# Da1yuqin/TCDiff

Hardware: AMD Instinct MI355X
Metric: sampled clips/sec (3 dancers x 150 frames, 1000 DDPM steps) (higher is better)
Workload: dtype bf16; 1 GPU; batch=16 clips/GPU, 3 dancers x 150 frames, 1000 DDPM steps (p_sample_loop, CFG w=2, cosine schedule), bf16, 1xMI355X; clips_per_gpu=16, ddpm_steps=1000

## Files before the change

include/tcdiff_hip.h:

```cpp
#ifndef TCDIFF_HIP_H
#define TCDIFF_HIP_H

#include <stdint.h>

#ifdef __cplusplus
extern "C" {
#endif

#ifndef __HIP__
typedef struct ihipStream_t* hipStream_t;
#endif

#define TCDIFF_OK 0
#define TCDIFF_ERR_ARG (-1)
#define TCDIFF_ERR_ALIGN (-2)
#define TCDIFF_ERR_LAUNCH (-3)
#define TCDIFF_ERR_UNSUPPORTED (-4)

#define TC_DTYPE_F32 0
#define TC_DTYPE_BF16 1
#define TC_DTYPE_BF16X3 2

#define TC_ACT_NONE 0
#define TC_ACT_RELU 1
// ... 6 lines not shown
#define TC_EPI_QKV_HEADS 2
#define TC_EPI_ATOMIC_F32 3

typedef struct {
    int mode;
    int act;
    float scale_q;
    const float* bias;
    void* out;
    void* out_k;
    void* out_v;
    int ldc;
    int L, Lp, H;
    int n_q, n_k;
    int tok_off;
    int seq_off;
    int k_splits;
    void* out2; int ldc2;
    const void* act_src; int ld_src;
    int act2;
    const int* drop_seed; int drop_site; uint32_t drop_thr; float drop_scale;
    int hgroup; long hgroup_stride;
    int small_m;
} tcdiff_tile_epi;

int tcdiff_gemm_tile(int dtype, const void* A, const void* A2, int split_n, const void* W, int M, int N, int K,
                     int lda, int ldw, int a_mod, const tcdiff_tile_epi* epi, hipStream_t stream);

#define TC_ROW_BIAS 1
#define TC_ROW_LN_POST 2
#define TC_ROW_FILM 4
#define TC_ROW_RES 8
#define TC_ROW_STORE_X 16
#define TC_ROW_NEXT_LN 32
#define TC_ROW_STORE_H 64
#define TC_ROW_STORE_ROT 128

typedef struct {
    int flags;
    const float* bias;
    const float* ln_g;
    const float* ln_b;
    float ln_eps;
    const float* film;
    int film_ld;
    const float* xres;
    int xres_mod;
// ... 433 lines not shown
```

tcdiff_amd/_lib.py:

```python
import ctypes as C
import os

HERE = os.path.dirname(os.path.abspath(__file__))
LIB_PATH = os.environ.get("TCDIFF_LIB_PATH") or os.path.join(HERE, "libtcdiff_gfx950.so")

DT_F32, DT_BF16, DT_BF16X3 = 0, 1, 2
ACT_NONE, ACT_RELU, ACT_GELU, ACT_MISH, ACT_SILU = 0, 1, 2, 3, 4
EPI_STORE_T, EPI_STORE_F32, EPI_QKV_HEADS = 0, 1, 2
ROW_BIAS, ROW_LN_POST, ROW_FILM, ROW_RES, ROW_STORE_X, ROW_NEXT_LN, ROW_STORE_H, ROW_STORE_ROT = \
    1, 2, 4, 8, 16, 32, 64, 128
SAMPLER_DDPM, SAMPLER_DDIM = 0, 1
EXPORT_NORMAL, EXPORT_LONG = 0, 1
SAMPLER_ADVANCE = 0x100
CHAIN_A, CHAIN_B, CHAIN_B_LAST, CHAIN_FULL, CHAIN_FULL_LAST, CHAIN_FRONT = 0, 1, 2, 3, 4, 5

_vp, _i, _f, _l = C.c_void_p, C.c_int, C.c_float, C.c_long


class TileEpi(C.Structure):
    _fields_ = [("mode", _i), ("act", _i), ("scale_q", _f), ("bias", _vp), ("out", _vp), ("out_k", _vp),
                ("out_v", _vp), ("ldc", _i), ("L", _i), ("Lp", _i), ("H", _i), ("n_q", _i), ("n_k", _i),
                ("tok_off", _i), ("seq_off", _i), ("k_splits", _i), ("out2", _vp), ("ldc2", _i), ("act_src", _vp),
                ("ld_src", _i), ("act2", _i), ("drop_seed", _vp), ("drop_site", _i), ("drop_thr", C.c_uint32),
                ("drop_scale", _f), ("hgroup", _i), ("hgroup_stride", _l), ("small_m", _i)]


class RowEpi(C.Structure):
    _fields_ = [("flags", _i), ("bias", _vp), ("ln_g", _vp), ("ln_b", _vp), ("ln_eps", _f), ("film", _vp),
                ("film_ld", _i), ("xres", _vp), ("xres_mod", _i), ("xout", _vp), ("L", _i), ("nln_g", _vp),
                ("nln_b", _vp), ("nln_eps", _f), ("hout", _vp), ("rout", _vp), ("rope", _vp), ("out_mul", _i),
                ("out_add", _i), ("groups", _i)]


class ChainArgs(C.Structure):
    _fields_ = [("mode", _i), ("n_stages", _i), ("M", _i), ("L", _i), ("a_mod", _i), ("xres_mod", _i), ("H", _i),
                ("Lp", _i), ("A", _vp), ("wstream", _vp), ("film", _vp), ("xres", _vp),
                ("xout", _vp), ("n2_g", _vp), ("n2_b", _vp), ("rope", _vp), ("q_out", _vp), ("b1", _vp),
                ("film3", _vp), ("n4_g", _vp), ("n4_b", _vp), ("b3", _vp), ("nn_g", _vp), ("nn_b", _vp),
                ("k_out", _vp), ("v_out", _vp), ("h_out", _vp), ("film_ld", _i), ("ln_eps", _f), ("n2_eps", _f),
                ("n4_eps", _f), ("nn_eps", _f), ("scale_q", _f), ("filmb", _vp),
                ("n3_g", _vp), ("n3_b", _vp), ("kf", _vp), ("vf", _vp), ("n_shared", _i), ("nkt", _i), ("Lk", _i),
                ("xres_rowmajor", _i), ("rope_rows", _i), ("dn", _i), ("mt", _i), ("out_ld", _i), ("nw", _i), ("seq_blocks", _i), ("sa_q", _vp), ("sa_kf", _vp), ("sa_vf", _vp),
                ("sa_nkt", _i), ("qf_out", _vp), ("kf_out", _vp), ("vf_out", _vp), ("out_nkt", _i)]


PROLOGUE_X, PROLOGUE_COND = 1, 2

# ... 45 lines not shown
                ("tap_blocks", _vp)]


class NavTrainArgs(C.Structure):
    _fields_ = [("seed0", C.c_uint32), ("seed1", C.c_uint32), ("drop_thr", C.c_uint32), ("drop_scale", _f), ("cond", _vp), ("x_in", _vp)] + \
        [(n, _vp) for n in ("lstm_gates", "lstm_c", "lstm_h", "xs", "xmid", "att_o", "lse", "hid", "dec_z", "mus_z", "d_out", "gx",
                            "g_dec", "g_mpb", "g_m", "g_hid", "g_a", "g_o", "delta", "g_qkv", "n1", "n2", "ln_part", "g_me", "g_mp",
                            "g_mz", "g_gates", "partial", "grads")]


class AdanScalars(C.Structure):
    _fields_ = [(n, _f) for n in ("b1", "omb1", "b2", "omb2", "b3", "omb3", "cm", "cv", "cn", "eps", "lr", "denom")] + \
        [("first", _i)]


class NavAdamWScalars(C.Structure):
    _fields_ = [(n, _f) for n in ("decay", "wd", "omb1", "beta2", "omb2", "neg_step", "bc2_sqrt", "eps")] + [("decoupled", _i)]


NAV_LOSS_BLOCK = 2048

_SIGS = {
    "tcdiff_gemm_tile": [_i, _vp, _vp, _i, _vp, _i, _i, _i, _i, _i, _i, C.POINTER(TileEpi), _vp],
    "tcdiff_gemm_rowln": [_i, _vp, _vp, _i, _i, _i, _i, _i, C.POINTER(RowEpi), _vp],
    "tcdiff_attention": [_i, _vp, _vp, _vp, _vp, _i, _i, _i, _i, _i, _i, _i, _i, _i, _vp],
    "tcdiff_q_sample_traj": [_vp, _vp, _vp, _vp, _vp, _vp, _i, _i, _i, _i, _vp],
    "tcdiff_ax_from_6v": [_vp, _l, _i, _l, _vp, _vp],
    "tcdiff_smpl_fk": [_vp, _vp, _l, C.POINTER(_i), C.POINTER(_f), _vp, _vp],
    "tcdiff_loss_terms": [_vp, _vp, _vp, _vp, _vp, _vp, _vp, _i, _i, _i, _i, _i, _vp],
    "tcdiff_adan_step": [_vp, _i, C.POINTER(AdanScalars), _vp],
    "tcdiff_pack_kv_frags": [_vp, _vp, _vp, _vp, _i, _i, _i, _i, _i, _i, _vp],
    "tcdiff_chain": [C.POINTER(ChainArgs), _vp],
    "tcdiff_chain_split": [C.POINTER(ChainArgs), _i, _vp, _vp, _vp],
    "tcdiff_ln_rot": [_i, _vp, _i, _vp, _vp, _f, _vp, _vp, _vp, _vp, _i, _i, _vp],
    "tcdiff_rope_table": [_vp, _vp, _i, _vp],
    "tcdiff_convert_pad": [_i, _vp, _vp, _i, _i, _i, _i, _l, _l, _vp],
    "tcdiff_sinusoidal": [_i, _vp, _i, _vp, _vp, _vp],
    "tcdiff_mean_pool": [_vp, _vp, _i, _i, _i, _vp],
    "tcdiff_add_act": [_i, _vp, _vp, _vp, _i, _i, _vp, _vp, _vp],
    "tcdiff_scatter_time_kv": [_i, _vp, _i, _vp, _vp, _vp, _i, _i, _i, _i, _i, _vp],
    "tcdiff_step_begin": [_vp, _vp, _vp, _i, _vp],
    "tcdiff_step_end": [_vp, _vp],
    "tcdiff_step_prologue": [_i, _vp, _vp],
    "tcdiff_sampler_update": [_i, _vp, _vp, _i, _vp, _vp, _vp, _vp, _i, _i, _i, _vp, _vp, _vp, C.c_uint64, _i, _vp],
    "tcdiff_window_couple": [_vp, _i, _i, _i, _vp],
    "tcdiff_window_couple_step": [_vp, _i, _i, _i, _vp, _vp, _vp],
# ... 97 lines not shown
```

tcdiff_amd/csrc/gemm.hip:

```cpp
#include "attn_common.h"
#include "train_common.h"
#include "tcdiff_hip.h"

#ifdef TC_STAMP
__device__ unsigned long long* g_tc_stamp = nullptr;
extern "C" int tcdiff_debug_stamp_buffer(void* p) {
    return hipMemcpyToSymbol(HIP_SYMBOL(g_tc_stamp), &p, sizeof(p)) == hipSuccess ? 0 : -1;
}
#define TC_STAMP_AT(i) do { if (tid == 0 && g_tc_stamp) g_tc_stamp[blockIdx.x * 8 + (i)] = __builtin_amdgcn_s_memrealtime(); } while (0)
#define TC_STAMP_W(i) do { if (lane == 0 && g_tc_stamp && (i) < 32) g_tc_stamp[blockIdx.x * 32 + (i)] = __builtin_amdgcn_s_memrealtime(); } while (0)
#else
#define TC_STAMP_AT(i) do { } while (0)
#define TC_STAMP_W(i) do { } while (0)
#endif

template <class P>
DEVINL void unpack_chunk(const u32x4& c, float (&v)[16 / sizeof(typename P::elem_t)]) {
    if (P::IS_BF16) {
#pragma unroll
        for (int j = 0; j < 4; ++j) {
            v[2 * j] = bf2f((uint16_t)(c[j] & 0xffffu));
            v[2 * j + 1] = bf2f((uint16_t)(c[j] >> 16));
        }
    } else {
// ... 692 lines not shown
        const f32x4_t b = *reinterpret_cast<const f32x4_t*>(e.bias + n);
#pragma unroll
        for (int t = 0; t < 4; ++t) v[t] += b[t];
    }
#pragma unroll
    for (int t = 0; t < 4; ++t) v[t] = apply_act(v[t], e.act);
    if (F32OUT) {
        *reinterpret_cast<f32x4_t*>(reinterpret_cast<float*>(e.out) + (long)m * e.ldc + n) = f32x4_t{v[0], v[1], v[2], v[3]};
    } else {
        uint2 pk = {pack_bf2(v[0], v[1]), pack_bf2(v[2], v[3])};
        *reinterpret_cast<uint2*>(reinterpret_cast<uint16_t*>(e.out) + (long)m * e.ldc + n) = pk;
    }
}

static bool small_product(int dtype, const void* A2, int M, int N, int K, const tcdiff_tile_epi& e, int n_cu) {
    static const bool off = [] { const char* v = getenv("TCDIFF_GEMM_SMALL"); return v && v[0] == '0'; }();
    if (off || !e.small_m || dtype != TC_DTYPE_BF16 || A2 || (e.mode != TC_EPI_STORE_T && e.mode != TC_EPI_STORE_F32) || e.out2 || e.act_src)
        return false;
    if (N % 32 || K % 32 || K > 2048 || e.ldc % 4 || (e.bias && !aligned16(e.bias))) return false;
    const long big = (long)((N + 127) / 128) * ((M + 127) / 128), small = (long)(N / 32) * ((M + 31) / 32);
    return big * 4 <= n_cu && small <= 2L * n_cu;
}

static int launch_tile(int dtype, const void* A, const void* A2, int split_n, const void* W, int M, int N, int K,
                       int lda, int ldw, int a_mod, const tcdiff_tile_epi* epi, hipStream_t stream) {
    if (!A || !W || !epi || M <= 0 || N <= 0 || K <= 0) return TC_ERR_ARG;
    if (dtype != TC_DTYPE_BF16 && dtype != TC_DTYPE_F32 && dtype != TC_DTYPE_BF16X3) return TC_ERR_ARG;
    if (dtype == TC_DTYPE_BF16X3 && (epi->mode == TC_EPI_ATOMIC_F32 || epi->out2 || epi->act_src)) return TC_ERR_UNSUPPORTED;
    if (dtype == TC_DTYPE_BF16X3 && epi->mode == TC_EPI_STORE_T && epi->ldc % 4) return TC_ERR_ARG;
    const int es = dtype == TC_DTYPE_BF16 ? 2 : 4;
    const int kt = dtype == TC_DTYPE_BF16 ? 64 : 32;
    if (K % kt != 0) return TC_ERR_ARG;
    if (!aligned16(A) || !aligned16(W) || (A2 && !aligned16(A2)) || ((long)lda * es) % 16 || ((long)ldw * es) % 16)
        return TC_ERR_ALIGN;
    if (A2 && (split_n % 128 != 0)) return TC_ERR_ARG;
    if ((long)(a_mod > 0 ? a_mod : M) * lda * es >= (1L << 32) || (long)N * ldw * es >= (1L << 32)) return TC_ERR_ARG;
    if (epi->bias && !aligned16(epi->bias)) return TC_ERR_ALIGN;
    if (epi->act < TC_ACT_NONE || epi->act > TC_ACT_SILU) return TC_ERR_ARG;
    if (epi->mode == TC_EPI_QKV_HEADS) {
        if (epi->L <= 0 || epi->Lp <= 0 || epi->H <= 0 || epi->n_q % 128 || epi->n_k % 128 || N % 64) return TC_ERR_ARG;
        if ((epi->n_q > 0 && (!epi->out || !aligned16(epi->out))) ||
            (epi->n_k > 0 && (!epi->out_k || !aligned16(epi->out_k))) ||
            (N > epi->n_q + epi->n_k && (!epi->out_v || !aligned16(epi->out_v))))
            return TC_ERR_ALIGN;
    } else {
        if (!epi->out) return TC_ERR_ARG;
// ... 21 lines not shown
        hipError_t err = hipSuccess;
#define TC_TILE_ATTR(POL, ACTK)                                                                                    \
        if (err == hipSuccess)                                                                                     \
            err = hipFuncSetAttribute(reinterpret_cast<const void*>(gemm_tile_kernel<POL, ACTK, 4>),              \
                                      hipFuncAttributeMaxDynamicSharedMemorySize, 4 * 2 * 128 * TC_ROWB);
        TC_TILE_ATTR(MmaBF16, 0) TC_TILE_ATTR(MmaBF16, 1) TC_TILE_ATTR(MmaBF16, 2) TC_TILE_ATTR(MmaBF16, 3)
        TC_TILE_ATTR(MmaF32, 0) TC_TILE_ATTR(MmaF32, 1) TC_TILE_ATTR(MmaF32, 2) TC_TILE_ATTR(MmaF32, 3)
        TC_TILE_ATTR(MmaBF16x3, 0) TC_TILE_ATTR(MmaBF16x3, 1) TC_TILE_ATTR(MmaBF16x3, 2) TC_TILE_ATTR(MmaBF16x3, 3)
#undef TC_TILE_ATTR
        return err;
    });
    if (n_cu < 0) return n_cu;
    if (small_product(dtype, A2, M, N, K, e, n_cu)) {
        const dim3 sgrid((unsigned)((N / 32) * ((M + 31) / 32)));
        if (e.mode == TC_EPI_STORE_F32)
            hipLaunchKernelGGL(gemm_small_kernel<true>, sgrid, dim3(512), 0, stream, (const char*)A, (const char*)W, M, N, K,
                               (long)lda * es, (long)ldw * es, a_mod, e);
        else
            hipLaunchKernelGGL(gemm_small_kernel<false>, sgrid, dim3(512), 0, stream, (const char*)A, (const char*)W, M, N, K,
                               (long)lda * es, (long)ldw * es, a_mod, e);
        TC_CHECK_LAUNCH();
        return TC_OK;
    }
    const bool deep = (long)grid.x * 4 <= (long)n_cu * 5 && K / kt / e.k_splits >= 3;
#define TC_LAUNCH_TILE(POL, ACTK)                                                                                       \
    if (deep)                                                                                                           \
        hipLaunchKernelGGL((gemm_tile_kernel<POL, ACTK, 4>), grid, dim3(256), 4 * 2 * 128 * TC_ROWB, stream,            \
                           (const char*)A, (const char*)A2, split_n, (const char*)W, M, N, K, (long)lda * es,           \
                           (long)ldw * es, a_mod, e);                                                                    \
    else                                                                                                                \
        hipLaunchKernelGGL((gemm_tile_kernel<POL, ACTK, 2>), grid, dim3(256), 2 * 2 * 128 * TC_ROWB, stream,            \
                           (const char*)A, (const char*)A2, split_n, (const char*)W, M, N, K, (long)lda * es,           \
                           (long)ldw * es, a_mod, e)
#define TC_DISPATCH_TILE(POL)                                      \
    switch (actk) {                                                \
        case 0: TC_LAUNCH_TILE(POL, 0); break;                     \
        case 1: TC_LAUNCH_TILE(POL, 1); break;                     \
        case 2: TC_LAUNCH_TILE(POL, 2); break;                     \
        default: TC_LAUNCH_TILE(POL, 3); break;                    \
    }
    if (dtype == TC_DTYPE_BF16) {
        TC_DISPATCH_TILE(MmaBF16)
    } else if (dtype == TC_DTYPE_BF16X3) {
        TC_DISPATCH_TILE(MmaBF16x3)
    } else {
        TC_DISPATCH_TILE(MmaF32)
    }
    TC_CHECK_LAUNCH();
    return TC_OK;
}

extern "C" int tcdiff_gemm_tile(int dtype, const void* A, const void* A2, int split_n, const void* W, int M, int N,
                                int K, int lda, int ldw, int a_mod, const tcdiff_tile_epi* epi,
                                hipStream_t stream) {
    if (epi && epi->mode == TC_EPI_ATOMIC_F32) return TC_ERR_ARG;
    return launch_tile(dtype, A, A2, split_n, W, M, N, K, lda, ldw, a_mod, epi, stream);
}

extern "C" int tcdiff_gemm_splitk(int dtype, const void* A, const void* W, int M, int N, int K, int lda, int ldw,
                                  float* out, int ldc, int splits, hipStream_t stream) {
    if (!out || ldc < N || splits < 1) return TC_ERR_ARG;
    tcdiff_tile_epi e = {};
    e.mode = TC_EPI_ATOMIC_F32;
    e.out = out;
    e.ldc = ldc;
    e.k_splits = splits;
    return launch_tile(dtype, A, nullptr, 0, W, M, N, K, lda, ldw, 0, &e, stream);
}

extern "C" int tcdiff_gemm_tn(int dtype, const void* A, const void* B, int M, int N, int K, int lda, int ldb, float* out,
                              int ldc, int splits, hipStream_t stream) {
    if (!A || !B || !out || M <= 0 || N <= 0 || K <= 0 || ldc < N || splits < 1 || lda < M || ldb < N) return TC_ERR_ARG;
// ... 131 lines not shown
```

tcdiff_amd/csrc/gemm_rows.hip:

```cpp
#include "chain_core.h"
#include "train_common.h"

struct RowsArgs {
    const char* A;
    const char* A2;
    const char* wstream;
    int split_n, n_stages, M, N, lda_bytes;
    tcdiff_tile_epi e;
};

DEVINL void unpack8(const u32x4& c, float (&v)[8]) {
#pragma unroll
    for (int i = 0; i < 4; ++i) {
        v[2 * i] = __builtin_bit_cast(float, c[i] << 16);
        v[2 * i + 1] = __builtin_bit_cast(float, c[i] & 0xFFFF0000u);
    }
}
DEVINL u32x4 pack8(const float (&v)[8]) {
    u32x4 c;
#pragma unroll
    for (int i = 0; i < 4; ++i) c[i] = pack_bf2(v[2 * i], v[2 * i + 1]);
    return c;
}

// ... 144 lines not shown
                    for (int t = 0; t < 8; ++t) f[t] = y[t] * gelu_grad(x[t]);
                } else if (e.act2 == ACT_RELU) {
#pragma unroll
                    for (int t = 0; t < 8; ++t) f[t] = x[t] > 0.0f ? y[t] : 0.0f;
                } else {
#pragma unroll
                    for (int t = 0; t < 8; ++t) f[t] = y[t] * act_grad(x[t], e.act2);
                }
                if (e.drop_thr) {
#pragma unroll
                    for (int t = 0; t < 8; ++t)
                        f[t] = drop_keep(dc, (uint32_t)m * (uint32_t)a.N + (uint32_t)(n + t)) ? f[t] : 0.0f;
                }
                *reinterpret_cast<u32x4*>(o1 + (long)m * e.ldc + n) = pack8(f);
            });
        } else {
            uint16_t* o1 = reinterpret_cast<uint16_t*>(e.out);
            staged_rows<MT>(acc, stg, lane, [&](int row, int ch, const u32x4& val) {
                const int m = m0 + row;
                if (m < M) *reinterpret_cast<u32x4*>(o1 + (long)m * e.ldc + col0 + 8 * ch) = val;
            });
        }
    }
}

__global__ __launch_bounds__(256) void pack_row_streams_kernel(const tcdiff_ws_desc* __restrict__ descs) {
    const tcdiff_ws_desc d = descs[blockIdx.y];
    const unsigned o = blockIdx.x * 256u + threadIdx.x;
    if (o >= (unsigned)d.N * (unsigned)(d.K >> 3)) return;
    const unsigned kst = (unsigned)d.K >> 5, np = (unsigned)d.N >> 9;
    const int c = o & 15, g = (o >> 4) & 3, nt = (o >> 6) & 3;
    const unsigned q = o >> 8;
    const unsigned ks = q % kst, p = (q / kst) % np, w = q / (kst * np);
    const int pg = (0x9C >> (2 * g)) & 3;
    const long n = 512 * (int)p + 64 * (int)w + 16 * nt + c, k0 = 32 * (int)ks + 8 * pg;
    const float* src = d.src + n * d.sn + k0 * d.sk;
    float v[8];
    if (d.sk == 1) {
        const f32x4_t a = ld4(src), b = ld4(src + 4);
        v[0] = a[0]; v[1] = a[1]; v[2] = a[2]; v[3] = a[3]; v[4] = b[0]; v[5] = b[1]; v[6] = b[2]; v[7] = b[3];
    } else {
#pragma unroll
        for (int j = 0; j < 8; ++j) v[j] = src[j * d.sk];
    }
    const unsigned long od = ((((unsigned long)w * d.np_dst + d.p0 + p) * d.kst_dst + d.ks0 + ks) << 8) + (o & 255u);
    reinterpret_cast<u32x4*>(d.dst)[od] = pack8(v);
// ... 43 lines not shown
    a.A = reinterpret_cast<const char*>(A);
    a.A2 = reinterpret_cast<const char*>(A2);
    a.wstream = reinterpret_cast<const char*>(wstream);
    a.split_n = split_n;
    a.n_stages = (N / 512) * (K / 32);
    a.M = M;
    a.N = N;
    a.lda_bytes = lda * 2;
    a.e = e;
    const dim3 grid((M + 16 * mt - 1) / (16 * mt));
#define ROWS_LAUNCH(KST_)                                                                                             \
    do {                                                                                                              \
        if (mt == 4) hipLaunchKernelGGL((gemm_rows_kernel<KST_, 4>), grid, dim3(512), CH_SMEM, stream, a);            \
        else if (mt == 2) hipLaunchKernelGGL((gemm_rows_kernel<KST_, 2>), grid, dim3(512), CH_SMEM, stream, a);       \
        else hipLaunchKernelGGL((gemm_rows_kernel<KST_, 1>), grid, dim3(512), CH_SMEM, stream, a);                    \
    } while (0)
    if (K == 512) ROWS_LAUNCH(16);
    else ROWS_LAUNCH(32);
#undef ROWS_LAUNCH
    TC_CHECK_LAUNCH();
    return TC_OK;
}

extern "C" int tcdiff_pack_row_streams(const tcdiff_ws_desc* descs_dev, int n_desc, int max_elems, hipStream_t stream) {
    if (!descs_dev || n_desc <= 0 || n_desc > 65535 || max_elems <= 0 || max_elems % 2048) return TC_ERR_ARG;
    hipLaunchKernelGGL(pack_row_streams_kernel, dim3((unsigned)(max_elems / 2048), (unsigned)n_desc), dim3(256), 0, stream, descs_dev);
    TC_CHECK_LAUNCH();
    return TC_OK;
}
```

tcdiff_amd/engine.py:

```python
from __future__ import annotations

import math
import os
from typing import Dict, Optional

import torch

from . import _lib as L
from . import kernels as K
from .form import Form, resolve_form

NL_FILM = 3


class DenoiserEngine:
    def __init__(self, cfg: dict, device: torch.device, compute: str = "bf16"):
        L.load()
        if device.type != "cuda":
            raise L.TcdiffError("DenoiserEngine needs a HIP device (cuda:N); there is no CPU fallback")
        self.cfg = dict(cfg)
        self.dev = device
        self.dt = K.dtype_id(compute)
        self.T = K.TORCH_DT[self.dt]
        self.kt = K.k_tile(self.dt)
# ... 8 lines not shown
        self.S, self.dn, self.nf, self.ff = c["seq_len"], c["dn"], c["nfeats"], c["ff"]
        self.Lseq = self.S * self.dn
        self.Lp = K.round_up(self.Lseq, 128)
        self.Lps = K.round_up(self.S, 128)
        self.Lpc = K.round_up(self.S + 2, 128)
        self.w: Dict[str, torch.Tensor] = {}
        self.weights_version = None
        self.plan_B = 0
        self.tables_key = None
        self.film_tab = None
        self._sampler_state = None
        self._side, self._forked = None, False
        self.last_form: Optional[Form] = None
        self.n_cu = torch.cuda.get_device_properties(device).multi_processor_count
        self.skt = (self.Lseq + 31) // 32
        self.act = int(cfg.get("act", L.ACT_GELU))
        self.abs_pos = bool(cfg.get("abs_pos", False))
        self.use_chain = self.dt == L.DT_BF16 and os.environ.get("TCDIFF_CHAIN", "1") != "0" and self.ff == 1024 \
            and self.H == 8 and self.act == L.ACT_GELU and not self.abs_pos
        self.use_full = self.use_chain and os.environ.get("TCDIFF_CHAIN", "2") == "2"
        self.nkt = (self.S + 2 + 31) // 32
        self.fold_in = self.dt == L.DT_BF16 and os.environ.get("TCDIFF_FOLD_IN", "1") != "0"
        self.kin = K.round_up(self.dn * self.nf, 64)
        self.fold_out = self.use_chain and os.environ.get("TCDIFF_FOLD_OUT", "1") != "0"
        self.front = self.use_full and os.environ.get("TCDIFF_FRONT", "1") != "0" and self.S >= 8
        self.fuse_sa = self.use_full and self.dt == L.DT_BF16 and os.environ.get("TCDIFF_FUSE_SA", "1") == "1"
        self.chain_nw = int(os.environ.get("TCDIFF_CHAIN_NW", "8"))
        if self.chain_nw not in (4, 8):
            raise L.TcdiffError("TCDIFF_CHAIN_NW must be 8 or 4")
        self.reset_graphs()

    def reset_graphs(self):
        self.graphs = {}
        self.graph_warm = set()
        self.generation = getattr(self, "generation", 0) + 1

    def sampler_state(self, n_steps: int, rows: int, nfeat: int):
        st = self._sampler_state
        if st is None or st["x"].shape != (rows, nfeat) or st["cap"] < n_steps:
            cap = max(4096, n_steps)
            dev = self.dev
            st = dict(cap=cap,
                      x=torch.zeros(rows, nfeat, device=dev), eps=torch.zeros(rows, nfeat, device=dev),
                      cval=torch.zeros(rows, nfeat, device=dev), qeps=torch.zeros(rows, nfeat, device=dev),
                      cmask=torch.zeros(rows, nfeat, device=dev),
                      traj=torch.zeros(rows, 3, device=dev), counter=torch.zeros(8, device=dev, dtype=torch.int32),
# ... 72 lines not shown
                    parts += [n512(qkv[0:512], n), n512(qkv[512:1024], n), n512(qkv[1024:1536], n)]
                return torch.cat(parts, 1)
            w[p + "chainA"], w[p + "chainB"] = chain_a(8).contiguous(), chain_b(8).contiguous()
            if self.use_full:
                w[p + "chainF"] = torch.cat([chain_a(nw), chain_b(nw)], 1).contiguous()

    def _f32(self, t: torch.Tensor) -> torch.Tensor:
        return t.detach().to(device=self.dev, dtype=torch.float32).contiguous()

    def load_weights(self, sd: Dict[str, torch.Tensor], version=None):
        w, f, p = {}, self._f32, self._pack
        g = lambda k: sd[k].detach()
        self.sd_f32 = lambda k: sd[k].detach().to(self.dev, torch.float32)
        w["in.w"], w["in.b"] = p(g("input_projection.weight"), 192), f(g("input_projection.bias"))
        for i, j in ((0, "f1"), (2, "f2"), (4, "f3")):
            w[j + ".w"] = p(g(f"relative_projection_layer.{i}.weight"))
            w[j + ".b"] = f(g(f"relative_projection_layer.{i}.bias"))
        if self.fold_in:
            W3 = g("relative_projection_layer.0.weight").to(self.dev, torch.float32).reshape(1024, self.dn, 512)
            Win = g("input_projection.weight").to(self.dev, torch.float32)
            bin_ = g("input_projection.bias").to(self.dev, torch.float32)
            w["f1in.w"] = p(torch.einsum("odk,kn->odn", W3, Win).reshape(1024, self.dn * self.nf), self.kin)
            w["f1in.b"] = (torch.einsum("odk,k->o", W3, bin_) + w["f1.b"]).contiguous()
        w["t1.w"], w["t1.b"] = p(g("time_mlp.1.weight")), f(g("time_mlp.1.bias"))
        w["tc.w"], w["tc.b"] = p(g("to_time_cond.0.weight")), f(g("to_time_cond.0.bias"))
        w["tt.w"], w["tt.b"] = p(g("to_time_tokens.0.weight")), f(g("to_time_tokens.0.bias"))
        w["null_embed"] = f(g("null_cond_embed")).reshape(self.S, 512)
        w["null_hidden"] = f(g("null_cond_hidden")).reshape(1, 512)
        w["nc.g"], w["nc.b"] = f(g("norm_cond.weight")), f(g("norm_cond.bias"))
        w["c0.w"], w["c0.b"] = p(g("cond_projection.0.weight")), f(g("cond_projection.0.bias"))
        w["c2.w"], w["c2.b"] = p(g("cond_projection.2.weight")), f(g("cond_projection.2.bias"))
        for i in range(2):
            q = f"cond_encoder.{i}."
            w[f"e{i}.qkv.w"], w[f"e{i}.qkv.b"] = p(g(q + "self_attn.in_proj_weight")), f(g(q + "self_attn.in_proj_bias"))
            w[f"e{i}.o.w"], w[f"e{i}.o.b"] = p(g(q + "self_attn.out_proj.weight")), f(g(q + "self_attn.out_proj.bias"))
            w[f"e{i}.l1.w"], w[f"e{i}.l1.b"] = p(g(q + "linear1.weight")), f(g(q + "linear1.bias"))
            w[f"e{i}.l2.w"], w[f"e{i}.l2.b"] = p(g(q + "linear2.weight")), f(g(q + "linear2.bias"))
            for n in ("norm1", "norm2"):
                w[f"e{i}.{n}.g"], w[f"e{i}.{n}.b"] = f(g(q + n + ".weight")), f(g(q + n + ".bias"))
        w["na.g"], w["na.b"] = f(g("non_attn_cond_projection.0.weight")), f(g("non_attn_cond_projection.0.bias"))
        w["na1.w"], w["na1.b"] = p(g("non_attn_cond_projection.1.weight")), f(g("non_attn_cond_projection.1.bias"))
        w["na3.w"], w["na3.b"] = p(g("non_attn_cond_projection.3.weight")), f(g("non_attn_cond_projection.3.bias"))
        film_w, film_b = [], []
        for l in range(self.NL):
            q = f"seqTransDecoder.stack.{l}."
            sa, ca = q + "self_attn.", q + "multihead_attn."
# ... 228 lines not shown
            with torch.cuda.stream(self._side):
                K.step_prologue(*args, parts=L.PROLOGUE_COND, **extra)
            self._forked = True
            return
        K.step_prologue(*args, **extra)
        if tab is None:
            K.gemm_tile(dt, b["film_in"], w["film.w"], n_rows_seq, nfilm, 512, bias=w["film.b"], mode=L.EPI_STORE_F32,
                        out=b["film"], ldc=nfilm)

    def network(self, x: torch.Tensor, B: int, branches: int, kv_slot0: int, n_shared: int, film_row0: int,
                x_ready: bool = False, form: Optional[Form] = None):
        dt, w, b = self.dt, self.w, self.b
        Lq, S, H, dn, NL = self.Lseq, self.S, self.H, self.dn, self.NL
        Rs, R = B * Lq, branches * B * Lq
        nseq = branches * B
        form = self.last_form = self.form(nseq) if form is None else form
        fld = NL * NL_FILM * 1024
        film0 = b["film"][film_row0:]
        rope = w["rope"]
        if not x_ready:
            K.convert_pad(dt, x, b["xin"], *self._xin_shape(Rs))
        sm = form.small_m
        if self.fold_in:
            K.gemm_tile(dt, b["xin"], w["f1in.w"], B * S, 1024, self.kin, bias=w["f1in.b"], act=L.ACT_RELU, out=b["f1"],
                        ldc=1024, small_m=sm)
        else:
            K.gemm_tile(dt, b["xin"], w["in.w"], Rs, 512, 192, bias=w["in.b"], out=b["xp"], ldc=512, small_m=sm)
            K.gemm_tile(dt, b["xp"], w["f1.w"], B * S, 1024, 512 * dn, bias=w["f1.b"], act=L.ACT_RELU, out=b["f1"],
                        ldc=1024, small_m=sm)
        K.gemm_tile(dt, b["f1"], w["f2.w"], B * S, 1024, 1024, bias=w["f2.b"], act=L.ACT_RELU, out=b["f2"], ldc=1024, small_m=sm)
        if form.frag_front:
            K.gemm_tile(dt, b["f2"], w["f3.w"], B * S, 512 * dn, 1024, bias=w["f3.b"], mode=L.EPI_STORE_F32, out=b["xs"],
                        ldc=512 * dn, small_m=True)
            K.chain(L.CHAIN_FRONT, Rs, Lq, None, w["front"][0], split_part=0, xres=b["xs"], nn_g=w["l0.norm1.g"],
                    nn_b=w["l0.norm1.b"], nn_eps=1e-5, rope=w["rope_cb"], qf_out=b["Qf"], kf_out=b["sKf"][0], vf_out=b["sVf"][0],
                    out_nkt=self.skt, scale_q=0.125, H=H)
        elif self.front:
            K.chain(L.CHAIN_FRONT, B * S, Lq, b["f2"], w["front"], b3=w["f3.b"], nn_g=w["l0.norm1.g"],
                    nn_b=w["l0.norm1.b"], nn_eps=1e-5, rope=w["rope_cb"], xout=b["xs"], q_out=b["Q"], k_out=b["K"],
                    v_out=b["V"], scale_q=0.125, Lp=self.Lp, H=H, dn=dn)
        elif self.abs_pos:
            K.gemm_rowln(dt, b["f2"], w["f3.w"], B * S, 1024, bias=w["f3.b"], xout=b["xs"], Lseq=Lq,
                         flags=L.ROW_BIAS | L.ROW_STORE_X, out_mul=dn, out_add=0, groups=dn)
            K.add_rows(b["xs"], 512, b["pe_x"], 512, b["xs"], 512, Rs, 512)
            K.ln_rot(dt, b["xs"], Rs, w["l0.norm1.g"], w["l0.norm1.b"], 1e-5, h=b["h"], rot=b["rot"], rope=rope, pos_mod=Lq)
        else:
            K.gemm_rowln(dt, b["f2"], w["f3.w"], B * S, 1024, bias=w["f3.b"], xout=b["xs"], Lseq=Lq,
                         flags=L.ROW_BIAS | L.ROW_STORE_X | L.ROW_NEXT_LN | L.ROW_STORE_H | L.ROW_STORE_ROT,
                         nln_g=w["l0.norm1.g"], nln_b=w["l0.norm1.b"], nln_eps=1e-5, hout=b["h"], rout=b["rot"],
                         rope=rope, out_mul=dn, out_add=0, groups=dn)
        Kc0 = b["Kc"][:, kv_slot0:]
        Vc0 = b["Vc"][:, kv_slot0:]
        if self._forked:
# ... 139 lines not shown
```

tcdiff_amd/kernels.py:

```python
import ctypes as C

import torch

from . import _lib as L

TORCH_DT = {L.DT_F32: torch.float32, L.DT_BF16: torch.bfloat16, L.DT_BF16X3: torch.float32}


def dtype_id(name_or_dtype) -> int:
    if isinstance(name_or_dtype, str) and name_or_dtype == "bf16x3":
        return L.DT_BF16X3
    if name_or_dtype in ("bf16", torch.bfloat16, L.DT_BF16):
        return L.DT_BF16
    if name_or_dtype in ("f32", "fp32", torch.float32, L.DT_F32):
        return L.DT_F32
    if name_or_dtype == L.DT_BF16X3 and not isinstance(name_or_dtype, bool):
        return L.DT_BF16X3
    raise ValueError(f"unsupported compute dtype {name_or_dtype!r} (bf16, f32 or bf16x3)")


def k_tile(dt: int) -> int:
    return 64 if dt == L.DT_BF16 else 32


# ... 14 lines not shown

def from_x3(t: torch.Tensor) -> torch.Tensor:
    q = t.contiguous().view(torch.int16).reshape(t.shape[:-1] + (t.shape[-1] // 4, 8))
    hi = q[..., :4].contiguous().view(torch.bfloat16).to(torch.float32)
    lo = q[..., 4:].contiguous().view(torch.bfloat16).to(torch.float32)
    return (hi + lo).reshape(t.shape)


def round_up(x: int, m: int) -> int:
    return (x + m - 1) // m * m


def stream() -> int:
    return torch.cuda.current_stream().cuda_stream


def _p(t):
    return None if t is None else t.data_ptr()


def gemm_tile(dt, A, W, M, N, K, *, lda=None, ldw=None, A2=None, split_n=0, a_mod=0, mode=L.EPI_STORE_T,
              act=L.ACT_NONE, bias=None, out=None, ldc=0, out_k=None, out_v=None, scale_q=1.0, Lseq=0, Lp=0, H=0,
              n_q=0, n_k=0, tok_off=0, seq_off=0, out2=None, ldc2=0, act_src=None, ld_src=0, act2=L.ACT_NONE, seed=None,
              site=0, thr=0, drop_scale=1.0, hgroup=0, hgroup_stride=0, small_m=False):
    lib = L.load()
    e = L.TileEpi(mode, act, scale_q, _p(bias), _p(out), _p(out_k), _p(out_v), ldc, Lseq, Lp, H, n_q, n_k, tok_off,
                  seq_off, 0, _p(out2), ldc2, _p(act_src), ld_src, act2, _p(seed), site, thr, drop_scale, hgroup, hgroup_stride,
                  int(bool(small_m)))
    rc = lib.tcdiff_gemm_tile(dt, _p(A), _p(A2), split_n, _p(W), M, N, K, lda if lda else K, ldw if ldw else K,
                              a_mod, C.byref(e), stream())
    L.check(rc, "tcdiff_gemm_tile")


def gemm_rows_ok(dt, N, K) -> bool:
    return dt == L.DT_BF16 and K in (512, 1024) and N > 0 and N % 512 == 0


def gemm_rows(A, wstream, M, N, K, *, lda=None, A2=None, split_n=0, mode=L.EPI_STORE_T, bias=None, out=None, ldc=0,
              out_k=None, out_v=None, scale_q=1.0, Lseq=0, Lp=0, H=0, n_q=0, n_k=0, out2=None, ldc2=0, act_src=None, ld_src=0,
              act2=L.ACT_NONE, seed=None, site=0, thr=0, drop_scale=1.0, mt=0):
    if tuple(wstream.shape) != (8, (N // 512) * (K // 32), 2048) or not wstream.is_contiguous():
        raise L.TcdiffError(f"weight stream of a [{N}, {K}] matrix must be contiguous [8, {(N // 512) * (K // 32)}, 2048], got "
                            f"{tuple(wstream.shape)}")
    e = L.TileEpi(mode, L.ACT_NONE, scale_q, _p(bias), _p(out), _p(out_k), _p(out_v), ldc, Lseq, Lp, H, n_q, n_k, 0, 0, 0,
                  _p(out2), ldc2, _p(act_src), ld_src, act2, _p(seed), site, thr, drop_scale, 0, 0)
    rc = L.load().tcdiff_gemm_rows(_p(A), _p(A2), split_n, _p(wstream), M, N, K, lda if lda else K, C.byref(e), mt, stream())
    L.check(rc, "tcdiff_gemm_rows")


def ws_table(entries, device):
    n = len(entries)
    arr = (L.WsDesc * n)()
    mx = 0
    for d, e in zip(arr, entries):
# ... 407 lines not shown
```

Before: 14.71 clips/s.

## Route fused input MLP GEMMs through pre-packed weight-stream kernel

Adds a streaming GEMM path in which each wave reads pre-packed weight fragments with buffer loads straight into registers while activation rows are staged in LDS. Launch_tile sends eligible bf16 STORE_T GEMMs with bias and ReLU there, and the engine pre-packs the f1in and f2 weights so the two 1024-wide front MLP GEMMs use it when not in small-M mode. The aim is to cut LDS staging of weights and raise MFMA issue efficiency for these large-N GEMMs, at the cost of extra packed weight memory and a new kernel whose tiling may not suit every M.

```diff
diff --git a/include/tcdiff_hip.h b/include/tcdiff_hip.h
--- a/include/tcdiff_hip.h
+++ b/include/tcdiff_hip.h
@@ -52,7 +52,13 @@
     const int* drop_seed; int drop_site; uint32_t drop_thr; float drop_scale;
     int hgroup; long hgroup_stride;
     int small_m;
+    const void* wstream;
 } tcdiff_tile_epi;
+
+#define TC_PLAN_TILE 0
+#define TC_PLAN_SMALL 1
+#define TC_PLAN_STREAM 2
+int tcdiff_gemm_tile_plan(int dtype, int M, int N, int K, const tcdiff_tile_epi* epi, int has_a2, int a_mod, int n_cu);
 
 int tcdiff_gemm_tile(int dtype, const void* A, const void* A2, int split_n, const void* W, int M, int N, int K,
                      int lda, int ldw, int a_mod, const tcdiff_tile_epi* epi, hipStream_t stream);
diff --git a/tcdiff_amd/_lib.py b/tcdiff_amd/_lib.py
--- a/tcdiff_amd/_lib.py
+++ b/tcdiff_amd/_lib.py
@@ -22,7 +22,7 @@
                 ("out_v", _vp), ("ldc", _i), ("L", _i), ("Lp", _i), ("H", _i), ("n_q", _i), ("n_k", _i),
                 ("tok_off", _i), ("seq_off", _i), ("k_splits", _i), ("out2", _vp), ("ldc2", _i), ("act_src", _vp),
                 ("ld_src", _i), ("act2", _i), ("drop_seed", _vp), ("drop_site", _i), ("drop_thr", C.c_uint32),
-                ("drop_scale", _f), ("hgroup", _i), ("hgroup_stride", _l), ("small_m", _i)]
+                ("drop_scale", _f), ("hgroup", _i), ("hgroup_stride", _l), ("small_m", _i), ("wstream", _vp)]
 
 
 class RowEpi(C.Structure):
@@ -114,6 +114,7 @@
 
 _SIGS = {
     "tcdiff_gemm_tile": [_i, _vp, _vp, _i, _vp, _i, _i, _i, _i, _i, _i, C.POINTER(TileEpi), _vp],
+    "tcdiff_gemm_tile_plan": [_i, _i, _i, _i, C.POINTER(TileEpi), _i, _i, _i],
     "tcdiff_gemm_rowln": [_i, _vp, _vp, _i, _i, _i, _i, _i, C.POINTER(RowEpi), _vp],
     "tcdiff_attention": [_i, _vp, _vp, _vp, _vp, _i, _i, _i, _i, _i, _i, _i, _i, _i, _vp],
     "tcdiff_q_sample_traj": [_vp, _vp, _vp, _vp, _vp, _vp, _i, _i, _i, _i, _vp],
diff --git a/tcdiff_amd/csrc/gemm.hip b/tcdiff_amd/csrc/gemm.hip
--- a/tcdiff_amd/csrc/gemm.hip
+++ b/tcdiff_amd/csrc/gemm.hip
@@ -738,6 +738,13 @@
     return big * 4 <= n_cu && small <= 2L * n_cu;
 }
 
+static bool stream_product(int dtype, bool has_a2, int a_mod, int N, int K, const tcdiff_tile_epi& e) {
+    if (!e.wstream || dtype != TC_DTYPE_BF16 || has_a2 || a_mod > 0 || e.mode != TC_EPI_STORE_T || e.out2 || e.act_src) return false;
+    if (e.act != TC_ACT_NONE && e.act != TC_ACT_RELU) return false;
+    return N > 0 && N % 512 == 0 && K >= 64 && K % 64 == 0 && K <= 1024 && e.ldc >= N && e.ldc % 8 == 0;
+}
+int tc_launch_gemm_stream(const void* A, int M, int N, int K, int lda, const tcdiff_tile_epi& e, hipStream_t stream);
+
 static int launch_tile(int dtype, const void* A, const void* A2, int split_n, const void* W, int M, int N, int K,
                        int lda, int ldw, int a_mod, const tcdiff_tile_epi* epi, hipStream_t stream) {
     if (!A || !W || !epi || M <= 0 || N <= 0 || K <= 0) return TC_ERR_ARG;
@@ -805,6 +812,7 @@
         TC_CHECK_LAUNCH();
         return TC_OK;
     }
+    if (stream_product(dtype, A2 != nullptr, a_mod, N, K, e)) return tc_launch_gemm_stream(A, M, N, K, lda, e, stream);
     const bool deep = (long)grid.x * 4 <= (long)n_cu * 5 && K / kt / e.k_splits >= 3;
 #define TC_LAUNCH_TILE(POL, ACTK)                                                                                       \
     if (deep)                                                                                                           \
@@ -831,6 +839,13 @@
     }
     TC_CHECK_LAUNCH();
     return TC_OK;
+}
+
+extern "C" int tcdiff_gemm_tile_plan(int dtype, int M, int N, int K, const tcdiff_tile_epi* epi, int has_a2, int a_mod, int n_cu) {
+    if (!epi || M <= 0 || N <= 0 || K <= 0 || n_cu <= 0) return TC_ERR_ARG;
+    if (dtype != TC_DTYPE_BF16 && dtype != TC_DTYPE_F32 && dtype != TC_DTYPE_BF16X3) return TC_ERR_ARG;
+    if (small_product(dtype, has_a2 ? epi : nullptr, M, N, K, *epi, n_cu)) return TC_PLAN_SMALL;
+    return stream_product(dtype, has_a2 != 0, a_mod, N, K, *epi) ? TC_PLAN_STREAM : TC_PLAN_TILE;
 }
 
 extern "C" int tcdiff_gemm_tile(int dtype, const void* A, const void* A2, int split_n, const void* W, int M, int N,
diff --git a/tcdiff_amd/csrc/gemm_rows.hip b/tcdiff_amd/csrc/gemm_rows.hip
--- a/tcdiff_amd/csrc/gemm_rows.hip
+++ b/tcdiff_amd/csrc/gemm_rows.hip
@@ -190,6 +190,117 @@
             });
         }
     }
+}
+
+struct StreamArgs {
+    const char* A;
+    const char* wstream;
+    const float* bias;
+    uint16_t* out;
+    int M, kst, ngrp, lda_bytes, ldc, relu;
+};
+
+template <int NG, int MT>
+DEVINL void phase_stream(f32x4_t (&acc)[4][MT], const char* abuf, WStream& ws, int lane, int kst) {
+    constexpr int NST = 4 * NG, RD = CH_D;
+    lane = fresh_v(lane);
+    const FragOff fo = frag_off(abuf, lane);
+    u32x4 b[MT];
+#pragma unroll
+    for (int mt = 0; mt < MT; ++mt) b[mt] = frag_rd(fo, 0, mt);
+    FragOff fo2 = fo;
+    if (NST > 16) {
+        fo2.e += 65536u;
+        fo2.o += 65536u;
+        asm volatile("" : "+v"(fo2.e), "+v"(fo2.o));
+    }
+    const bool cut = kst < NST;
+#pragma unroll
+    for (int ks = 0; ks < NST; ++ks) {
+        const int i = ks % RD;
+        u32x4 wv[4];
+#pragma unroll
+        for (int nt = 0; nt < 4; ++nt) wv[nt] = ws.w[i][nt];
+        if (ks + RD < NST) ws_load(ws, i, (unsigned)(ks + RD));
+        u32x4 nb[MT];
+#pragma unroll
+        for (int mt = 0; mt < MT; ++mt) nb[mt] = b[mt];
+        if (ks + 1 < NST) {
+            const FragOff& fn = ks + 1 < 16 ? fo : fo2;
+            const int kl = (ks + 1) & 15;
+#pragma unroll
+            for (int mt = 0; mt < MT; ++mt) nb[mt] = frag_rd(fn, kl, mt);
+        }
+        __builtin_amdgcn_sched_barrier(0);
+        if (!(ks >= NST - 2 && cut)) {
+#pragma unroll
+            for (int mt = 0; mt < MT; ++mt) {
+#pragma unroll
+                for (int nt = 0; nt < 4; ++nt) mma16(acc[nt][mt], wv[nt], b[mt]);
+            }
+        }
+        __builtin_amdgcn_sched_barrier(0);
+        acc_fence(acc);
+        frag_fence(nb);
+#pragma unroll
+        for (int mt = 0; mt < MT; ++mt) b[mt] = nb[mt];
+    }
+    ws.pos = NST;
+}
+
+template <int NG, int MT>
+__global__ __launch_bounds__(512) void gemm_stream_kernel(StreamArgs a) {
+    constexpr int BR = 16 * MT;
+    extern __shared__ __attribute__((aligned(16))) char smem[];
+    const int tid = threadIdx.x, lane = tid & 63;
+    const int wave = __builtin_amdgcn_readfirstlane(tid >> 6);
+    const int blk = xcd_remap(blockIdx.x, gridDim.x);
+    const int rb = blk / a.ngrp, grp = blk - rb * a.ngrp;
+    const int m0 = rb * BR, M = a.M;
+    char* abuf = smem + CH_ABUF;
+
+    if (wave < 2 * MT) {
+        const int nkt = a.kst >> 1;
+#pragma unroll 1
+        for (int kt = 0; kt < nkt; ++kt)
+            stage_glds<BR, 2 * MT>(abuf + kt * 8192, a.A + kt * TC_ROWB, a.lda_bytes, m0, M, 0, wave, lane);
+    }
+    WStream ws;
+    ws.rsrc = __builtin_amdgcn_make_buffer_rsrc(const_cast<char*>(a.wstream) + ((long)wave * a.ngrp + grp) * a.kst * CH_STAGE, 0,
+                                                a.kst * CH_STAGE, 0x00020000);
+    ws.voff = (unsigned)lane * 16u;
+    ws.pos = 0;
+    ws.last = (unsigned)a.kst - 1;
+#pragma unroll
+    for (int i = 0; i < CH_D; ++i) ws_load(ws, i, (unsigned)i);
+    __builtin_amdgcn_s_waitcnt(0x0F70);
+    __syncthreads();
+
+    f32x4_t acc[4][MT];
+    zero(acc);
+    phase_stream<NG, MT>(acc, abuf, ws, lane, a.kst);
+    const int col0 = 512 * grp + 64 * wave;
+    const int g = fresh_v(lane) >> 4;
+    if (a.bias) {
+#pragma unroll
+        for (int nt = 0; nt < 4; ++nt) {
+            const f32x4_t b4 = ld4(a.bias + col0 + 16 * nt + 4 * g);
+#pragma unroll
+            for (int mt = 0; mt < MT; ++mt) acc[nt][mt] += b4;
+        }
+    }
+    if (a.relu) {
+#pragma unroll
+        for (int nt = 0; nt < 4; ++nt)
+#pragma unroll
+            for (int mt = 0; mt < MT; ++mt)
+#pragma unroll
+                for (int t = 0; t < 4; ++t) acc[nt][mt][t] = fmaxf(acc[nt][mt][t], 0.0f);
+    }
+    staged_rows<MT>(acc, stage_area(smem, wave), lane, [&](int row, int ch, const u32x4& val) {
+        const int m = m0 + row;
+        if (m < M) *reinterpret_cast<u32x4*>(a.out + (long)m * a.ldc + col0 + 8 * ch) = val;
+    });
 }
 
 __global__ __launch_bounds__(256) void pack_row_streams_kernel(const tcdiff_ws_desc* __restrict__ descs) {
@@ -279,6 +390,48 @@
     return TC_OK;
 }
 
+#define TC_STREAM_MT 2
+int tc_launch_gemm_stream(const void* A, int M, int N, int K, int lda, const tcdiff_tile_epi& e, hipStream_t stream) {
+    if (!rows_al16(e.wstream)) return TC_ERR_ALIGN;
+    if (N % 512 || K % 64 || K < 64 || K > 1024 || e.ldc < N || e.ldc % 8) return TC_ERR_UNSUPPORTED;
+    static tc_dev_state dev_state;
+    const int n_cu = tc_device_once(dev_state, [](int) {
+        const void* fns[8] = {reinterpret_cast<const void*>(gemm_stream_kernel<1, TC_STREAM_MT>), reinterpret_cast<const void*>(gemm_stream_kernel<2, TC_STREAM_MT>),
+                              reinterpret_cast<const void*>(gemm_stream_kernel<3, TC_STREAM_MT>), reinterpret_cast<const void*>(gemm_stream_kernel<4, TC_STREAM_MT>),
+                              reinterpret_cast<const void*>(gemm_stream_kernel<5, TC_STREAM_MT>), reinterpret_cast<const void*>(gemm_stream_kernel<6, TC_STREAM_MT>),
+                              reinterpret_cast<const void*>(gemm_stream_kernel<7, TC_STREAM_MT>), reinterpret_cast<const void*>(gemm_stream_kernel<8, TC_STREAM_MT>)};
+        for (const void* f : fns) {
+            hipError_t er = hipFuncSetAttribute(f, hipFuncAttributeMaxDynamicSharedMemorySize, CH_SMEM);
+            if (er != hipSuccess) return er;
+        }
+        return hipSuccess;
+    });
+    if (n_cu < 0) return n_cu;
+    StreamArgs a;
+    a.A = reinterpret_cast<const char*>(A);
+    a.wstream = reinterpret_cast<const char*>(e.wstream);
+    a.bias = e.bias;
+    a.out = reinterpret_cast<uint16_t*>(e.out);
+    a.M = M;
+    a.kst = K / 32;
+    a.ngrp = N / 512;
+    a.lda_bytes = lda * 2;
+    a.ldc = e.ldc;
+    a.relu = e.act == TC_ACT_RELU;
+    constexpr int BR = 16 * TC_STREAM_MT;
+    const long nblk = (long)((M + BR - 1) / BR) * a.ngrp;
+    if (nblk >= (1L << 31)) return TC_ERR_ARG;
+    const dim3 grid((unsigned)nblk);
+#define STREAM_CASE(NG_) case NG_: hipLaunchKernelGGL((gemm_stream_kernel<NG_, TC_STREAM_MT>), grid, dim3(512), CH_SMEM, stream, a); break
+    switch ((a.kst + 3) / 4) {
+        STREAM_CASE(1); STREAM_CASE(2); STREAM_CASE(3); STREAM_CASE(4); STREAM_CASE(5); STREAM_CASE(6); STREAM_CASE(7); STREAM_CASE(8);
+        default: return TC_ERR_UNSUPPORTED;
+    }
+#undef STREAM_CASE
+    TC_CHECK_LAUNCH();
+    return TC_OK;
+}
+
 extern "C" int tcdiff_pack_row_streams(const tcdiff_ws_desc* descs_dev, int n_desc, int max_elems, hipStream_t stream) {
     if (!descs_dev || n_desc <= 0 || n_desc > 65535 || max_elems <= 0 || max_elems % 2048) return TC_ERR_ARG;
     hipLaunchKernelGGL(pack_row_streams_kernel, dim3((unsigned)(max_elems / 2048), (unsigned)n_desc), dim3(256), 0, stream, descs_dev);
diff --git a/tcdiff_amd/engine.py b/tcdiff_amd/engine.py
--- a/tcdiff_amd/engine.py
+++ b/tcdiff_amd/engine.py
@@ -54,6 +54,7 @@
         self.nkt = (self.S + 2 + 31) // 32
         self.fold_in = self.dt == L.DT_BF16 and os.environ.get("TCDIFF_FOLD_IN", "1") != "0"
         self.kin = K.round_up(self.dn * self.nf, 64)
+        self.fusion_stream = self.fold_in and os.environ.get("TCDIFF_FUSION_STREAM", "1") != "0"
         self.fold_out = self.use_chain and os.environ.get("TCDIFF_FOLD_OUT", "1") != "0"
         self.front = self.use_full and os.environ.get("TCDIFF_FRONT", "1") != "0" and self.S >= 8
         self.fuse_sa = self.use_full and self.dt == L.DT_BF16 and os.environ.get("TCDIFF_FUSE_SA", "1") == "1"
@@ -172,6 +173,8 @@
             bin_ = g("input_projection.bias").to(self.dev, torch.float32)
             w["f1in.w"] = p(torch.einsum("odk,kn->odn", W3, Win).reshape(1024, self.dn * self.nf), self.kin)
             w["f1in.b"] = (torch.einsum("odk,k->o", W3, bin_) + w["f1.b"]).contiguous()
+            if self.fusion_stream:
+                w["f1in.ws"], w["f2.ws"] = K.stream_rows(w["f1in.w"]), K.stream_rows(w["f2.w"])
         w["t1.w"], w["t1.b"] = p(g("time_mlp.1.weight")), f(g("time_mlp.1.bias"))
         w["tc.w"], w["tc.b"] = p(g("to_time_cond.0.weight")), f(g("to_time_cond.0.bias"))
         w["tt.w"], w["tt.b"] = p(g("to_time_tokens.0.weight")), f(g("to_time_tokens.0.bias"))
@@ -446,13 +449,16 @@
             K.convert_pad(dt, x, b["xin"], *self._xin_shape(Rs))
         sm = form.small_m
         if self.fold_in:
+            ws1, ws2 = (w["f1in.ws"], w["f2.ws"]) if self.fusion_stream and not sm else (None, None)
             K.gemm_tile(dt, b["xin"], w["f1in.w"], B * S, 1024, self.kin, bias=w["f1in.b"], act=L.ACT_RELU, out=b["f1"],
-                        ldc=1024, small_m=sm)
+                        ldc=1024, small_m=sm, wstream=ws1)
         else:
+            ws2 = None
             K.gemm_tile(dt, b["xin"], w["in.w"], Rs, 512, 192, bias=w["in.b"], out=b["xp"], ldc=512, small_m=sm)
             K.gemm_tile(dt, b["xp"], w["f1.w"], B * S, 1024, 512 * dn, bias=w["f1.b"], act=L.ACT_RELU, out=b["f1"],
                         ldc=1024, small_m=sm)
-        K.gemm_tile(dt, b["f1"], w["f2.w"], B * S, 1024, 1024, bias=w["f2.b"], act=L.ACT_RELU, out=b["f2"], ldc=1024, small_m=sm)
+        K.gemm_tile(dt, b["f1"], w["f2.w"], B * S, 1024, 1024, bias=w["f2.b"], act=L.ACT_RELU, out=b["f2"], ldc=1024, small_m=sm,
+                    wstream=ws2)
         if form.frag_front:
             K.gemm_tile(dt, b["f2"], w["f3.w"], B * S, 512 * dn, 1024, bias=w["f3.b"], mode=L.EPI_STORE_F32, out=b["xs"],
                         ldc=512 * dn, small_m=True)
diff --git a/tcdiff_amd/kernels.py b/tcdiff_amd/kernels.py
--- a/tcdiff_amd/kernels.py
+++ b/tcdiff_amd/kernels.py
@@ -60,14 +60,37 @@
 def gemm_tile(dt, A, W, M, N, K, *, lda=None, ldw=None, A2=None, split_n=0, a_mod=0, mode=L.EPI_STORE_T,
               act=L.ACT_NONE, bias=None, out=None, ldc=0, out_k=None, out_v=None, scale_q=1.0, Lseq=0, Lp=0, H=0,
               n_q=0, n_k=0, tok_off=0, seq_off=0, out2=None, ldc2=0, act_src=None, ld_src=0, act2=L.ACT_NONE, seed=None,
-              site=0, thr=0, drop_scale=1.0, hgroup=0, hgroup_stride=0, small_m=False):
+              site=0, thr=0, drop_scale=1.0, hgroup=0, hgroup_stride=0, small_m=False, wstream=None):
+    if wstream is not None and (tuple(wstream.shape) != (8, (N // 512) * (K // 32), 2048) or wstream.element_size() != 2
+                                or not wstream.is_contiguous() or N % 512 or K % 32):
+        raise L.TcdiffError(f"weight stream of a [{N}, {K}] matrix must be contiguous 2-byte [8, (N / 512) (K / 32), 2048], got "
+                            f"{tuple(wstream.shape)}")
     lib = L.load()
     e = L.TileEpi(mode, act, scale_q, _p(bias), _p(out), _p(out_k), _p(out_v), ldc, Lseq, Lp, H, n_q, n_k, tok_off,
                   seq_off, 0, _p(out2), ldc2, _p(act_src), ld_src, act2, _p(seed), site, thr, drop_scale, hgroup, hgroup_stride,
-                  int(bool(small_m)))
+                  int(bool(small_m)), _p(wstream))
     rc = lib.tcdiff_gemm_tile(dt, _p(A), _p(A2), split_n, _p(W), M, N, K, lda if lda else K, ldw if ldw else K,
                               a_mod, C.byref(e), stream())
     L.check(rc, "tcdiff_gemm_tile")
+
+
+PLAN_TILE, PLAN_SMALL, PLAN_STREAM = 0, 1, 2
+
+
+def gemm_tile_plan(dt, M, N, K, *, mode=L.EPI_STORE_T, act=L.ACT_NONE, small_m=False, wstream=False, A2=False, a_mod=0, out2=False,
+                   act_src=False, ldc=None, n_cu=256) -> int:
+    e = L.TileEpi()
+    e.mode, e.act, e.small_m, e.ldc = mode, act, int(bool(small_m)), N if ldc is None else ldc
+    e.wstream, e.out2, e.act_src = (16 if wstream else None), (16 if out2 else None), (16 if act_src else None)
+    return L.load().tcdiff_gemm_tile_plan(dt, M, N, K, C.byref(e), int(bool(A2)), a_mod, n_cu)
+
+
+def stream_rows(W: torch.Tensor) -> torch.Tensor:
+    N, K_ = W.shape
+    if N % 512 or K_ % 32:
+        raise L.TcdiffError("stream_rows: N % 512 == 0 and K % 32 == 0")
+    w7 = W.reshape(N // 512, 8, 4, 16, K_ // 32, 4, 8)[:, :, :, :, :, [0, 3, 1, 2], :]
+    return w7.permute(1, 0, 4, 2, 5, 3, 6).reshape(8, (N // 512) * (K_ // 32), 2048).contiguous()
 
 
 def gemm_rows_ok(dt, N, K) -> bool:
```

Measured after the change: 14.61 clips/s. Within noise of the previous version (-0.7%).
